# FROL256/ada-ray-tracer

Hardware: AMD Instinct MI355X
Metric: Mrays/s (higher is better)
Workload: dtype f32; 1 GPU; C4: synthetic 1000000 triangles + 3 sphere lights in the Cornell box, 1920x1080, PT_MIS depth 8, 2x2 AA, 256 spp per step; parallelism=pixel-tiles x1, bvh_width=4, bvh_nodes=383662, bvh_max_stack=36

## Files before the change

### ada-ray-tracer_amd/csrc/art_api.cpp

```cpp
#include <hip/hip_runtime.h>
#include <rccl/rccl.h>

#include <algorithm>
#include <chrono>
#include <cstdio>
#include <cstdlib>
#include <cstring>
#include <mutex>
#include <string>
#include <vector>

#include "art_api_internal.h"
#include "art_lbvh.h"

namespace art {

Ctx g_devs[kMaxDevices];
int g_ndev = 1;
Ctx* g_cur = &g_devs[0];
std::mutex g_mu;
static ncclComm_t g_comms[kMaxDevices];
static bool g_comms_ready = false;
static EventPairs g_reduce_pairs;
static double g_reduce_ms = 0.0; static int g_reduces = 0, g_reduce_path = 0;
// ... 530 lines not shown
        for (DevPaths& b : bank) { b.P = pn * sn; b.npix = pn; b.pixmap = (const uint32_t*)c.b_pixmap.p + px0; b.sample_base = (uint32_t)(c.spp + s0); }
        carve(bank, bank[0].P, p->max_depth, c.opt.trace_kernel == TRACE_COOP);
        int trial = 0, shade_per = c.opt.opt_shade_per ? c.opt.opt_shade_per : (c.auto_phase >= 4 ? c.auto_per : 4);
        if (c.opt.opt_shade_per == 0 && c.auto_phase < 3 && c.opt.trace_kernel == TRACE_COOP) {
          const int64_t Pb = (int64_t)pn * sn;
          if (c.auto_phase == 0) c.auto_phase = 1;
          else if (c.auto_phase == 1) { trial = 1; c.auto_ms[0] = 0.0; c.auto_P[0] = Pb; c.auto_phase = 2; }
          else if (Pb == c.auto_P[0]) { trial = 2; shade_per = 2; c.auto_ms[1] = 0.0; c.auto_P[1] = Pb; c.auto_phase = 3; }
          else if (++c.auto_redo > 3) { c.auto_per = 4; c.auto_phase = 4; }
          else { trial = 1; c.auto_gen += 1; c.auto_ms[0] = 0.0; c.auto_P[0] = Pb; }
        }
        const bool dedup = c.opt.camera_dedup && !c.opt.count_tests && c.opt.trace_kernel == TRACE_COOP;
        const int cam_u = p->aa_on ? 4 : 1;
        const int cam_n = dedup ? cam_u * pn : bank[0].P;
        c.camera_traced += (uint64_t)cam_n;
        if (c.opt.trace_kernel == TRACE_COOP) {
          if (!c.d_live) HIP_TRY(hipMalloc(&c.d_live, 32 * 18 * sizeof(int)));
          unsigned long long* const rays_b = c.opt.count_tests ? c.d_counters + CNT_TRACED : nullptr;
          bank[0].rec_mode = REC_EXT;
          DevPaths q = bank[0];
          q.slot_id = nullptr;
          q.cam_dedup = dedup ? cam_u : 0;
          DevPaths qgen = q; qgen.P = cam_n;
          if (!c.d_items) { HIP_TRY(hipMalloc(&c.d_items, 32 * sizeof(unsigned long long))); HIP_TRY(hipMemsetAsync(c.d_items, 0, 32 * sizeof(unsigned long long), c.stream)); }
          { EventPairs::Timer t; HIP_TRY(c.stage_pairs.begin(t, c.stream, ev_tag(2))); launch_raygen(c.stream, F, c.scene, qgen); }
          launch_bump(c.stream, c.d_counters + CNT_RAYS, rays_b, (unsigned long long)q.P);
          { const RecordQueue rq = {cam_n, nullptr, 1}; TraceLaunch t = launch; t.records = &rq; if (trace(q, cam_n, t)) return 1; }
          for (int b = 0; b < p->max_depth; ++b) {
            const int in = b & 1, out = in ^ 1;
            const DevPaths& qi = (b == 0) ? q : bank[in];
            const bool last = b + 1 >= p->max_depth;
            bank[out].rec_mode = (p->render_type == ART_PT_STUPID) ? REC_EXT : (last ? REC_SHADOW : REC_BOTH);
            int* const n_in = c.d_live + 32 * b; int* const n_out = c.d_live + 32 * (b + 1);
            HIP_TRY(hipMemsetAsync(n_out, 0, sizeof(int), c.stream));
            { EventPairs::Timer t; HIP_TRY(c.stage_pairs.begin(t, c.stream, ev_tag(1, trial)));
              launch_shade_compact(c.stream, F, c.scene, qi, bank[out], b, b == 0 ? nullptr : n_in, n_out,
                                   const_cast<uint32_t*>(bank[out].slot_id), c.d_counters + CNT_LOST, c.d_counters + CNT_RAYS, rays_b, shade_per); }
            if (b == 0 && c.inject_lost) { launch_bump(c.stream, c.d_counters + CNT_LOST, nullptr, 1ull); c.inject_lost = 0; }
            if (g_debug_live) {
              int n = -1; unsigned long long r0 = 0;
              (void)hipStreamSynchronize(c.stream); (void)hipMemcpy(&n, n_out, 4, hipMemcpyDeviceToHost); (void)hipMemcpy(&r0, c.d_counters + CNT_RAYS, 8, hipMemcpyDeviceToHost);
              std::fprintf(stderr, "stage %d: items out %d of %d, rays so far %llu\n", b, n, q.P, r0);
            }
            if (!last || p->render_type != ART_PT_STUPID) {
              const RecordQueue rq = {-1, n_out, bank[out].rec_mode == REC_BOTH ? 2 : 1};
              TraceLaunch t = launch; t.item_count = n_out; t.records = &rq;
              if (trace(bank[out], 2 * q.P, t)) return 1;
            }
          }
          const int last = p->max_depth & 1;
          EventPairs::Timer fold_timer;
          HIP_TRY(c.stage_pairs.begin(fold_timer, c.stream, ev_tag(3)));
          launch_resolve_last(c.stream, bank[last], c.d_live + 32 * p->max_depth, p->max_depth - 1);
          if (bank[last].fold_dense) launch_fold_levels(c.stream, F, bank[last], p->max_depth, c.d_live);
          else launch_fold(c.stream, F, bank[last]);
          launch_accumulate(c.stream, F, q, sn, accum_ptr());
          HIP_TRY(fold_timer.end());
          launch_acc_items(c.stream, c.d_live, p->max_depth, q.P, c.d_items);
          c.stage.batches += 1;
        } else {
          DevPaths q = bank[0];
          q.slot_id = nullptr;
          q.final_flags = q.flags;
          launch_raygen(c.stream, F, c.scene, q);
          for (int b = 0; b < p->max_depth; ++b) {
            if (trace(q, b == 0 ? q.P : 2 * q.P, launch)) return 1;
            launch_shade(c.stream, F, c.scene, q, b);
          }
          if (p->render_type != ART_PT_STUPID) { if (trace(q, 2 * q.P, launch)) return 1; }
          launch_finish(c.stream, F, q, p->max_depth - 1);
          launch_accumulate(c.stream, F, q, sn, accum_ptr());
        }
        HIP_TRY(hipGetLastError());
      }
    }
  }
  HIP_TRY(pass_timer.end());
  if (clock) HIP_TRY(hipLaunchHostFunc(c.stream, clock_cb, &clock->t1));
  c.spp += S;
  c.stats.samples += (uint64_t)npix * S;
  if (spp_inout) *spp_inout = c.spp;
  return 0;
}

static int synchronize_one();
int synchronize() {
  Dev0Guard guard;
  int rc = 0;
  for (int k = 0; k < g_ndev; ++k) { if (use_dev(k) || synchronize_one()) rc = 1; }
  if (g_devs[0].device_ready && !use_dev(0)) fold_reduce_events();
  return rc;
}
static int synchronize_one() {
  Ctx& c = g_ctx;
  if (!c.device_ready) return 0;
  HIP_TRY(hipStreamSynchronize(c.stream));
  HIP_TRY(c.pass_pairs.fold(true, [&c](float ms, uint8_t) { c.stats.pass_ms += ms; }));
  if (collect_timing()) return 1;
  if (sync_updates()) return 1;
  if (c.stats.lost_paths != c.lost_reported) {
    const uint64_t n = c.stats.lost_paths - c.lost_reported;
    c.lost_reported = c.stats.lost_paths;
    return fail("render self-check: " + std::to_string(n) + " path(s) lost by the wavefront stages (ArtStats::lost_paths); the image is not valid");
  }
  return 0;
}

// ... 475 lines not shown
int art_get_stage_stats(ArtStageStats* out) {
  std::lock_guard<std::mutex> lk(g_mu);
  if (!out) return fail("null ArtStageStats");
  if (synchronize()) return 1;
  *out = g_devs[0].stage;
  return 0;
}

int art_get_stats(ArtStats* out) {
  std::lock_guard<std::mutex> lk(g_mu);
  if (!out) return fail("null stats");
  if (synchronize()) return 1;
  *out = g_devs[0].stats;
  for (int k = 1; k < g_ndev; ++k) {
    const ArtStats& t = g_devs[k].stats;
    out->rays += t.rays; out->samples += t.samples; out->box_tests += t.box_tests; out->tri_tests += t.tri_tests;
    out->node_visits += t.node_visits; out->leaf_visits += t.leaf_visits; out->traced_rays += t.traced_rays;
    out->lost_paths += t.lost_paths;
    out->pass_ms = std::max(out->pass_ms, t.pass_ms);
  }
  return 0;
}

int art_get_camera_rays_traced(uint64_t* out) {
  std::lock_guard<std::mutex> lk(g_mu);
  if (!out) return fail("null camera ray count");
  *out = 0;
  for (int k = 0; k < g_ndev; ++k) *out += g_devs[k].camera_traced;
  return 0;
}

static int set_option_one(const std::string& n, int64_t value);
int art_set_option(const char* name, int64_t value) {
  std::lock_guard<std::mutex> lk(g_mu);
  if (!name) return fail("null option");
  const std::string n(name);
  Ctx* const saved = g_cur;
  int rc = 0;
  for (int k = 0; k < g_ndev && !rc; ++k) { g_cur = &g_devs[k]; rc = set_option_one(n, value); }
  g_cur = saved;
  return rc;
}
static int set_option_one(const std::string& n, int64_t value) {
  if (n == "trace_kernel") { if (value != TRACE_COOP && value != TRACE_SIMPLE) return fail("trace_kernel: 0 (cooperative) or 1 (simple)"); g_ctx.opt.trace_kernel = (int)value; }
  else if (n == "queue_segments") { if (value != 1 && value != 2 && value != 4 && value != 8) return fail("queue_segments: 1, 2, 4 or 8"); g_ctx.opt.queue_segments = (int)value; }
  else if (n == "batch_paths") { if (value < 1024 || value > (1ll << 27)) return fail("batch_paths: 1024..2^27 (2 rays per path slot; the trace kernel addresses a ray's 16-byte hit record by a 32-bit byte offset)"); g_ctx.opt.batch_paths = value; g_ctx.auto_phase = 0; g_ctx.auto_redo = 0; g_ctx.auto_gen += 1; }
  else if (n == "paths_spread") { if (value < -1 || value > 65536) return fail("paths_spread: chunk size in MB, 0 = off (plain hipMalloc), -1 = automatic"); g_ctx.opt.paths_spread_mb = (int)value; release_paths(g_ctx); }
  else if (n == "spread_fail_at") { g_ctx.spread_fail_at = (int)value; release_paths(g_ctx); }
  else if (n == "inject_lost") { g_ctx.inject_lost = value != 0; }
  else if (n == "blocks_per_cu") { g_ctx.opt.opt_blocks_per_cu = (int)value; g_ctx.blocks_per_cu = 0; }
  else if (n == "query_slice") { if (value < 1 || value > (1ll << 28)) return fail("query_slice: 1 .. 2^28 rays per slice of a device query"); g_ctx.opt.query_slice = value; }
  else if (n == "count_tests") { g_ctx.opt.count_tests = value != 0; }
  else if (n == "camera_dedup") { if (value != 0 && value != 1) return fail("camera_dedup: 0 (every sample's camera ray is traced) or 1 (each distinct camera ray once per batch)"); g_ctx.opt.camera_dedup = value != 0; }
  else if (n == "shadow_anyhit") { g_ctx.opt.shadow_anyhit = value != 0; }
  else if (n == "skip_null_shadow") { g_ctx.opt.skip_null_shadow = value != 0; }
  else if (n == "inst_coop") { g_ctx.opt.inst_coop = value != 0; }
  else if (n == "shade_per") { if (value != 0 && value != 2 && value != 4) return fail("shade_per: 0 (measured), 2 or 4"); g_ctx.opt.opt_shade_per = (int)value; }
  else if (n == "ray_chunk") { if (value < 16 || value > 4096 || (value & 15)) return fail("ray_chunk: a multiple of 16, 16..4096"); g_ctx.opt.ray_chunk = (int)value; }
  else if (n == "refill_min") { if (value < 1 || value > 8) return fail("refill_min: 1..8"); g_ctx.opt.refill_min = (int)value; }
  else if (n == "node_min") { if (value < 0 || value > 8) return fail("node_min: 1..8, 0 = automatic"); g_ctx.opt.node_min = (int)value; }
  else if (n == "bvh_width") { if (value != 4 && value != 8) return fail("bvh_width: 4 or 8"); g_ctx.opt.bvh_params.width = (int)value; }
  else if (n == "lds_stack_cap") { if (value < 0 || value > kStackEntries) return fail("lds_stack_cap: 0 (automatic) .. 160"); g_ctx.opt.lds_stack_cap = (int)value; }
  else if (n == "bvh_max_leaf") { if (value < 0 || value > kMaxLeafTris) return fail("bvh_max_leaf: 1..8, 0 = defaults"); g_ctx.opt.bvh_params.max_leaf = value ? (int)value : BvhBuildParams().max_leaf; g_ctx.opt.bvh_params.gpu_max_leaf = (int)value; }
  else if (n == "inst_open") { if (value < 0 || value > 4096) return fail("inst_open: 1 .. 4096 entry points per instance, 0 = chosen from the instances' overlap"); g_ctx.opt.bvh_params.inst_open = (int)value; }
  else if (n == "bvh_spatial_splits") { g_ctx.opt.bvh_params.spatial_alpha = value ? 1.0e-5f : -1.0f; }
  else if (n == "bvh_builder") { if (value < 0 || value > 3) return fail("bvh_builder: 0 host SAH, 1 GPU LBVH, 2 GPU PLOC, 3 GPU SAH"); g_ctx.opt.bvh_params.builder = (int)value; }
  else if (n == "bvh_ploc_radius") { if (value < 1 || value > 64) return fail("bvh_ploc_radius: 1..64"); g_ctx.opt.bvh_params.ploc_radius = (int)value; }
  else if (n == "bvh_leaf_base_milli") { g_ctx.opt.bvh_params.leaf_base = (float)value / 1000.0f; }
  else if (n == "bvh_tri_cost_milli") { g_ctx.opt.bvh_params.tri_cost = (float)value / 1000.0f; }
  else if (n == "bvh_node_cost_milli") { g_ctx.opt.bvh_params.node_cost = (float)value / 1000.0f; }
  else return fail("unknown option " + n);
  return 0;
}

const char* art_last_error(void) { t_err = g_err; return t_err.c_str(); }

void art_shutdown(void) { std::lock_guard<std::mutex> lk(g_mu); shutdown(); }

}
```

### ada-ray-tracer_amd/csrc/art_api_internal.h

```cpp
#pragma once
#include <hip/hip_runtime.h>
#include <mutex>
#include <string>
#include <vector>
#include "../../include/art_hip.h"
#include "art_event_pairs.h"
#include "art_host_scene.h"
#include "art_kernels.h"

namespace art {

constexpr int kMaxDevices = 16;
constexpr int kCursorInts = 32 * 9;

struct DevBuf {
  void* p = nullptr; size_t bytes = 0;
  std::vector<hipMemGenericAllocationHandle_t> chunks; size_t chunk_bytes = 0, reserved = 0;
  void release();
};

struct UpdateLane {
  EventPairs pairs;
  hipEvent_t ready_ev = nullptr, done_ev = nullptr;
  DevBuf b_stage;
  bool unread = false;
  uint64_t bad_last = 0; bool bad_reported = true;
};

struct Options {
  int trace_kernel = TRACE_COOP;
  int64_t batch_paths = 128ll << 20;
  int opt_blocks_per_cu = 0;
  bool count_tests = false;
  bool camera_dedup = true;
  int node_min = 0;
  int refill_min = 2;
  int queue_segments = 8;
  int ray_chunk = 48;
  bool shadow_anyhit = true;
  bool skip_null_shadow = false;
  bool inst_coop = true;
  int opt_shade_per = 0;
  int lds_stack_cap = 0;
  int paths_spread_mb = -1;
  int64_t query_slice = 1ll << 24;
  BvhBuildParams bvh_params;
};

enum Counter {
  CNT_RAYS = 0,
  CNT_STATS = 3, CNT_TRACED = 7,
  CNT_NODE_ITERS = 8, CNT_LEAF_ITERS = 9, CNT_WAVE_ITERS = 10, CNT_LOST = 15, kCounters = 16
};

struct Ctx {
  int device = -1; bool device_ready = false; int num_cus = 0; int lds_per_cu = 160 * 1024; std::string arch;
  hipStream_t stream = nullptr;
  hipStream_t own_stream = nullptr;
  bool scene_ready = false;
  HostScene host_scene;
  DevScene scene;
  DevScene* d_scene = nullptr;
  DevBuf b_spheres, b_sphere_mat, b_lights, b_materials, b_bf_pos, b_bf_nrm, b_bf_uv, b_bf_idx, b_nodes, b_qnodes, b_tris, b_qtris, b_m_shade;
  int bvh_stack_bound = 8;
  int width = 0, height = 0, spp = 0;
  int rank = 0, nranks = 1, tile = 32, npix_local = 0;
  DevBuf b_inst, b_tlas_nodes, b_tlas_tris, b_blas_nodes, b_blas_tris;
  DevBuf b_accum, b_screen, b_stage, b_pixmap, b_paths, b_rays, b_ids, b_queue, b_ovf;
  DevBuf b_query;
  hipEvent_t q_ev[2] = {nullptr, nullptr};
  struct RefitPlan {
    bool ready = false;
    DevBuf b_idx, b_levels, b_tight, b_bad;
    std::vector<int> level_off;
    uint64_t bad_total = 0;
    UpdateLane lane;
  } refit;
  struct MovePlan {
    bool ready = false;
    DevBuf b_plan, b_work;
    MoveArgs args = MoveArgs();
    std::vector<int> level_off; const int32_t* levels = nullptr;
    bool small_entries = false;
    UpdateLane lane;
    struct Mesh { int32_t tri_base = -1, n_recs = 0, shade_base = 0, n_prims = 0; int64_t nverts = 0; const int32_t* idx = nullptr; int level_first = 0, level_end = 0; };
    std::vector<Mesh> meshes;
    std::vector<int> blas_level_off; const int32_t* blas_levels = nullptr;
    UpdateLane refit_lane;
  } move;
  int* d_live = nullptr;
  DevBuf b_reduced;
// ... 82 lines not shown
```

### ada-ray-tracer_amd/csrc/art_kernels.h

```cpp
#pragma once
#include <hip/hip_runtime.h>
#include "art_shade.h"
#include "art_qnode.h"
#include "art_instanced.h"

namespace art {

enum { TRACE_COOP = 0, TRACE_SIMPLE = 1 };

struct TraceArgs {
  int32_t n_rays;
  int32_t stack_entries;
  int32_t width;
  int32_t instanced;
  int32_t stack_overflow;
  int32_t segments;
  int32_t node_min;
  int32_t refill_min;
  const float* ray_ox; const float* ray_oy; const float* ray_oz;
  const float* ray_dx; const float* ray_dy; const float* ray_dz;
  const float* ray_tfar;
  float4* rec;
  const float* sh_min; int32_t shadow_begin;
  DevHit* hit;
  const DevInstance* inst; int32_t inst_shift;
  float* sh_t;
  const float* nodes; const uint32_t* qnodes; const float* tris; const float* qtris; int32_t n_tris;
  int32_t chunk;
  int* cursor;
  int* queue; int* queue_count;
  int32_t queue_fixed; const int* queue_items; int32_t queue_mul;
  int* ovf_queue; int* ovf_count;
  unsigned long long* stats;
  unsigned long long* live_rays;
  const int* item_count;
};

constexpr int kTraceRecBytes = 64;

void launch_raygen(hipStream_t st, const DevFrame& F, const DevScene& S, const DevPaths& Q);
void launch_bump(hipStream_t st, unsigned long long* a, unsigned long long* b, unsigned long long n);
void launch_acc_items(hipStream_t st, const int* live, int depth, int P, unsigned long long* items);
void launch_shade(hipStream_t st, const DevFrame& F, const DevScene& S, const DevPaths& Q, int bounce);
void launch_finish(hipStream_t st, const DevFrame& F, const DevPaths& Q, int last_level);
void launch_shade_compact(hipStream_t st, const DevFrame& F, const DevScene& S, const DevPaths& Qi, const DevPaths& Qo, int bounce,
                          const int* n_in, int* n_out, uint32_t* slot_out, unsigned long long* lost, unsigned long long* rays_a, unsigned long long* rays_b,
                          int per = 0);
void launch_resolve_last(hipStream_t st, const DevPaths& Q, const int* n, int last_level);
void launch_fold(hipStream_t st, const DevFrame& F, const DevPaths& Q);
void launch_fold_levels(hipStream_t st, const DevFrame& F, const DevPaths& Q, int max_depth, const int* counts);
void launch_accumulate(hipStream_t st, const DevFrame& F, const DevPaths& Q, int samples_in_batch, float* accum);
void launch_resolve(hipStream_t st, const float* accum, int n_pixels, float norm_c, uint32_t* screen);
void launch_debug(hipStream_t st, const DevFrame& F, const DevScene& S, const DevPaths& Q, float* accum, int32_t* prim_index, int32_t* mat_id, int32_t* prim_type);
void launch_to_xmajor_f3(hipStream_t st, const float* src, float* dst, int w, int h);
void launch_to_xmajor_u32(hipStream_t st, const uint32_t* src, uint32_t* dst, int w, int h);
void launch_from_xmajor_f3(hipStream_t st, const float* src, float* dst, int w, int h);
void launch_trace_instanced(hipStream_t st, const InstScene& T, const float* o, const float* d, const float* tfar, int n, InstHit* out);
void launch_pad_tris(hipStream_t st, const float* src12, float* dst16, int n);
void launch_add_f32(hipStream_t st, const float* src, float* dst, size_t n);
size_t trace_coop_lds_bytes(int stack_entries, int width);
void launch_trace(hipStream_t st, const DevScene* d_scene, const TraceArgs& A, int kernel, bool stats, int grid_blocks);
void launch_analytic(hipStream_t st, const DevScene& scene, const TraceArgs& A, bool stats);
int  trace_coop_blocks_per_cu(int stack_entries, int width);

constexpr int kArtHitWords = 11;
struct QueryArgs {
  int32_t n;
  const float* o3; const float* d3;
  const float* tnear; const float* tfar;
  float *ox, *oy, *oz, *dx, *dy, *dz, *tf;
  float* shm;
  DevHit* hit;
  uint32_t* out;
  uint8_t* occluded;
};
void launch_query_pack(hipStream_t st, const QueryArgs& Q);
void launch_query_finalize(hipStream_t st, const DevScene& S, const QueryArgs& Q);
void launch_query_occluded(hipStream_t st, const QueryArgs& Q);

constexpr float kRefitMaxCoord = 1.0e18f;
struct RefitArgs {
  const float* pos3f; const float* nrm3f;
  const int32_t* idx;
  int64_t nverts; int32_t n_prims, n_recs;
  float* tris; float* qtris; float* m_shade;
  unsigned long long* bad;
  float* nodes; QNode* qnodes;
  float* tight;
  int32_t width; float inflate_rel, inflate_abs;
};
void launch_refit_tris(hipStream_t st, const RefitArgs& R);
void launch_refit_level(hipStream_t st, const RefitArgs& R, const int32_t* level_nodes, int n);

struct GatherArgs {
  const float* pos3f; const int32_t* idx;
  int64_t nverts; int32_t n_prims;
  float* tri9;
  unsigned long long* bad;
};
void launch_gather_tri9(hipStream_t st, const GatherArgs& G);
void launch_tree_cost(hipStream_t st, const float* nodes, int n_nodes, int width, double* sums4);

struct MoveArgs {
// ... 36 lines not shown
```

### ada-ray-tracer_amd/csrc/art_kernels.hip

```cpp
#include <hip/hip_runtime.h>
#include <algorithm>
#include <type_traits>
#include "art_kernels.h"

namespace art {

template <int CTRL>
__device__ __forceinline__ int dpp_i(int v) { return __builtin_amdgcn_update_dpp(0, v, CTRL, 0xf, 0xf, true); }

constexpr int DPP_XOR1 = 0xB1;
constexpr int DPP_XOR2 = 0x4E;
constexpr int DPP_XOR3 = 0x1B;
constexpr int DPP_HALF_MIRROR = 0x141;

__device__ __forceinline__ int xor4_i(int v) { return dpp_i<DPP_XOR3>(dpp_i<DPP_HALF_MIRROR>(v)); }

template <int G> __device__ __forceinline__ int group_rank_g(int key);
template <> __device__ __forceinline__ int group_rank_g<4>(int key) {
  int r = 0;
  r += (dpp_i<DPP_XOR1>(key) < key);
  r += (dpp_i<DPP_XOR2>(key) < key);
  r += (dpp_i<DPP_XOR3>(key) < key);
  return r;
}
// ... 735 lines not shown
    const int r = wave * 64 + lane;
    const int n_all_k = s_nall[k], n_keep_k = s_nkeep[k], out0_k = s_out0[k];
    const int wo = r < n_keep_k ? base + out0_k + r : -1;
    if (r < n_all_k) {
      const uint2 hk = s_hint[k * 256 + r];
      const int w = c0 + k * 256 + (int)(hk.y & 255u);
      ItemHint ih; ih.key = hk.x; ih.mat = (hk.y & 256u) ? (int32_t)(hk.y >> 9) : -1;
      StageCtx cy = tables;
      if (staged) {
        const int nk = min(64, max(0, n_keep_k - wave * 64)), per = (Qo.rec_mode == REC_BOTH) ? 2 : 1;
        const size_t first = (size_t)per * (size_t)(base + out0_k + wave * 64);
        cy.stage = s_stage[wave]; cy.stage_pitch = kStagePitch; cy.stage_item = lane; cy.stage_count = nk; cy.lost = lost;
        cy.rec_base[0] = first; cy.rec_base[1] = (per == 2) ? first + (size_t)nk : first;
      }
      n_rays += shade_item(F, S, Qi, Qo, w, wo, bounce, lost, cy, &ih, CAMERA ? 1 : 0, 1);
    }
  }
  ART_TPROBE(tables.tprobe, 68);
#if defined(ART_TIME_PROBE)
  __syncthreads();
  if (threadIdx.x < 64 && s_tacc[threadIdx.x] != 0) atomicAdd(&g_lane_probe[2 * 64 + threadIdx.x], s_tacc[threadIdx.x]);
#endif
  if (Qo.rec != nullptr && rays_a != nullptr) {
    for (int off = 32; off > 0; off >>= 1) n_rays += __shfl_xor(n_rays, off);
    if (lane == 0 && n_rays) atomicAdd(&s_rays, n_rays);
    __syncthreads();
    if (threadIdx.x == 0 && s_rays) { atomicAdd(rays_a, (unsigned long long)s_rays); if (rays_b) atomicAdd(rays_b, (unsigned long long)s_rays); }
  }
}

__global__ void k_bump(unsigned long long* a, unsigned long long* b, unsigned long long n) { *a += n; if (b) *b += n; }
__global__ void k_acc_items(const int* live, int depth, int P, unsigned long long* items) {
  unsigned long long in = (unsigned long long)P;
  for (int b = 0; b < depth && b < 16; ++b) { const unsigned long long out = (unsigned long long)live[32 * (b + 1)]; items[b] += in; items[16 + b] += out; in = out; }
}

__global__ __launch_bounds__(256) void k_resolve_last(const DevPaths Q, const int* __restrict__ n_ptr, int last_level) {
  const int w = blockIdx.x * blockDim.x + threadIdx.x;
  if (w < *n_ptr) resolve_last_shadow(Q, w, last_level);
}
__global__ __launch_bounds__(256) void k_fold(const DevFrame F, const DevPaths Q) {
  const int slot = blockIdx.x * blockDim.x + threadIdx.x;
  if (slot < Q.P) fold_slot(F, Q, slot);
}

__global__ __launch_bounds__(256) void k_fold_level(const DevFrame F, const DevPaths Q, int level, int deepest, const int* __restrict__ n_ptr,
                                                    const float* __restrict__ nxt_r, const float* __restrict__ nxt_g, const float* __restrict__ nxt_b,
                                                    float* __restrict__ cur_r, float* __restrict__ cur_g, float* __restrict__ cur_b) {
  const int w = blockIdx.x * blockDim.x + threadIdx.x;
  const int n = n_ptr ? *n_ptr : Q.P;
  if (w < n) fold_level_item(F, Q, level, w, deepest != 0, nxt_r, nxt_g, nxt_b, cur_r, cur_g, cur_b);
}

__global__ __launch_bounds__(256) void k_finish(const DevFrame F, const DevPaths Q, int last_level) {
  const int slot = blockIdx.x * blockDim.x + threadIdx.x;
  if (slot < Q.P) finish_slot(F, Q, slot, last_level);
}

__global__ __launch_bounds__(256) void k_accumulate(const DevFrame F, const DevPaths Q, int samples_in_batch, float* accum) {
  const int pl = blockIdx.x * blockDim.x + threadIdx.x;
  if (pl < Q.npix) accumulate_pixel(F, Q, pl, samples_in_batch, accum);
}

__global__ __launch_bounds__(256) void k_resolve(const float* accum, int n_pixels, float norm_c, uint32_t* screen) {
  const int i = blockIdx.x * blockDim.x + threadIdx.x;
  if (i < n_pixels) screen[i] = resolve_pixel(mk3(accum[3 * (size_t)i], accum[3 * (size_t)i + 1], accum[3 * (size_t)i + 2]), norm_c);
}

__global__ __launch_bounds__(256) void k_debug(const DevFrame F, const DevScene S, const DevPaths Q, float* accum,
                                               int32_t* prim_index, int32_t* mat_id, int32_t* prim_type) {
  const int slot = blockIdx.x * blockDim.x + threadIdx.x;
  if (slot >= Q.P) return;
  uint32_t pixel, sample;
  slot_to_sample(Q, slot, pixel, sample);
  const DevHit hq = Q.hit[slot];
  const uint32_t key = hq.key;
  f3 col = mk3(0.0f, 0.0f, 0.0f);
  int32_t pi = -1, mi = -1, pt = -1;
  if (key != KEY_MISS) {
    const f3 o = mk3(Q.ray_ox[slot], Q.ray_oy[slot], Q.ray_oz[slot]), d = mk3(Q.ray_dx[slot], Q.ray_dy[slot], Q.ray_dz[slot]);
    const Surface sf = surface_at(S, o, d, hq.t, key, hq.u, hq.v);
    col = debug_palette(sf.mat_id);
    mi = sf.mat_id; pi = (int32_t)(key & KEY_INDEX_MASK);
    const uint32_t cls = key & ~KEY_INDEX_MASK;
    pt = (cls == KEY_CORNELL) ? 0 : (cls == KEY_SPHERE) ? 1 : (cls == KEY_QUAD) ? 3 : 2;
  }
  accum[3 * (size_t)pixel] = col.x; accum[3 * (size_t)pixel + 1] = col.y; accum[3 * (size_t)pixel + 2] = col.z;
  if (prim_index) prim_index[pixel] = pi;
  if (mat_id) mat_id[pixel] = mi;
  if (prim_type) prim_type[pixel] = pt;
}

__global__ __launch_bounds__(256) void k_to_xmajor_f3(const float* src_rowmajor, float* dst_xmajor, int w, int h) {
  const int i = blockIdx.x * blockDim.x + threadIdx.x;
  if (i >= w * h) return;
  const int x = i / h, y = i - x * h;
  const size_t s = (size_t)y * w + x;
  dst_xmajor[3 * (size_t)i] = src_rowmajor[3 * s]; dst_xmajor[3 * (size_t)i + 1] = src_rowmajor[3 * s + 1]; dst_xmajor[3 * (size_t)i + 2] = src_rowmajor[3 * s + 2];
}
__global__ __launch_bounds__(256) void k_to_xmajor_u32(const uint32_t* src_rowmajor, uint32_t* dst_xmajor, int w, int h) {
  const int i = blockIdx.x * blockDim.x + threadIdx.x;
  if (i >= w * h) return;
  const int x = i / h, y = i - x * h;
  dst_xmajor[i] = src_rowmajor[(size_t)y * w + x];
}
__global__ __launch_bounds__(256) void k_from_xmajor_f3(const float* src_xmajor, float* dst_rowmajor, int w, int h) {
// ... 14 lines not shown
__global__ __launch_bounds__(256) void k_add_f32(const float* __restrict__ src, float* __restrict__ dst, size_t n) {
  const size_t i = (size_t)blockIdx.x * blockDim.x + threadIdx.x;
  if (i < n) dst[i] = src[i] + dst[i];
}

static inline int blocks_for(int n) { return (n + 255) / 256; }

void launch_raygen(hipStream_t st, const DevFrame& F, const DevScene& S, const DevPaths& Q) {
  hipLaunchKernelGGL(k_raygen, dim3(blocks_for(Q.P)), dim3(256), 0, st, F, S, Q);
}
void launch_shade(hipStream_t st, const DevFrame& F, const DevScene& S, const DevPaths& Q, int bounce) {
  hipLaunchKernelGGL(k_shade, dim3(blocks_for(Q.P)), dim3(256), 0, st, F, S, Q, bounce);
}
#if defined(ART_LANE_PROBE)
__global__ void k_probe_on(int v) { g_lane_probe_on = v; }
#endif
void launch_shade_compact(hipStream_t st, const DevFrame& F, const DevScene& S, const DevPaths& Qi, const DevPaths& Qo, int bounce,
                          const int* n_in, int* n_out, uint32_t* slot_out, unsigned long long* lost, unsigned long long* rays_a, unsigned long long* rays_b,
                          int per) {
  const bool camera = Qi.synth0 && Qi.slot_id == nullptr;
  const int per_now = (per == 2) ? 2 : kShadePerThread;
  const dim3 grid((Qi.P + 256 * per_now - 1) / (256 * per_now));
#if defined(ART_LANE_PROBE)
  hipLaunchKernelGGL(k_probe_on, dim3(1), dim3(1), 0, st, 1);
#endif
  ShadeKernArgs A; A.F = F; A.S = S; A.Qi = Qi; A.Qo = Qo; A.bounce = bounce; A.n_in_ptr = n_in; A.n_out_ptr = n_out; A.slot_out = slot_out; A.lost = lost; A.rays_a = rays_a; A.rays_b = rays_b;
  if (per_now == 2) {
    if (camera) hipLaunchKernelGGL((k_shade_compact<2, true>), grid, dim3(256), 0, st, A);
    else hipLaunchKernelGGL((k_shade_compact<2, false>), grid, dim3(256), 0, st, A);
  } else {
    if (camera) hipLaunchKernelGGL((k_shade_compact<kShadePerThread, true>), grid, dim3(256), 0, st, A);
    else hipLaunchKernelGGL((k_shade_compact<kShadePerThread, false>), grid, dim3(256), 0, st, A);
  }
#if defined(ART_LANE_PROBE)
  hipLaunchKernelGGL(k_probe_on, dim3(1), dim3(1), 0, st, 0);
#endif
}
void launch_acc_items(hipStream_t st, const int* live, int depth, int P, unsigned long long* items) { hipLaunchKernelGGL(k_acc_items, dim3(1), dim3(1), 0, st, live, depth, P, items); }
void launch_bump(hipStream_t st, unsigned long long* a, unsigned long long* b, unsigned long long n) { hipLaunchKernelGGL(k_bump, dim3(1), dim3(1), 0, st, a, b, n); }
void launch_resolve_last(hipStream_t st, const DevPaths& Q, const int* n, int last_level) {
  hipLaunchKernelGGL(k_resolve_last, dim3(blocks_for(Q.P)), dim3(256), 0, st, Q, n, last_level);
}
void launch_fold(hipStream_t st, const DevFrame& F, const DevPaths& Q) {
  hipLaunchKernelGGL(k_fold, dim3(blocks_for(Q.P)), dim3(256), 0, st, F, Q);
}
void launch_fold_levels(hipStream_t st, const DevFrame& F, const DevPaths& Q, int max_depth, const int* counts) {
  for (int k = max_depth - 1; k >= 0; --k) {
    float* cur[3] = {(k & 1) ? Q.term_r : Q.rad_r, (k & 1) ? Q.term_g : Q.rad_g, (k & 1) ? Q.term_b : Q.rad_b};
    const float* nxt[3] = {(k & 1) ? Q.rad_r : Q.term_r, (k & 1) ? Q.rad_g : Q.term_g, (k & 1) ? Q.rad_b : Q.term_b};
    hipLaunchKernelGGL(k_fold_level, dim3(blocks_for(Q.P)), dim3(256), 0, st, F, Q, k, k == max_depth - 1 ? 1 : 0, k == 0 ? nullptr : counts + 32 * k,
                       nxt[0], nxt[1], nxt[2], cur[0], cur[1], cur[2]);
  }
}
void launch_finish(hipStream_t st, const DevFrame& F, const DevPaths& Q, int last_level) {
  hipLaunchKernelGGL(k_finish, dim3(blocks_for(Q.P)), dim3(256), 0, st, F, Q, last_level);
}
void launch_accumulate(hipStream_t st, const DevFrame& F, const DevPaths& Q, int samples_in_batch, float* accum) {
  hipLaunchKernelGGL(k_accumulate, dim3(blocks_for(Q.npix)), dim3(256), 0, st, F, Q, samples_in_batch, accum);
}
void launch_resolve(hipStream_t st, const float* accum, int n_pixels, float norm_c, uint32_t* screen) {
  hipLaunchKernelGGL(k_resolve, dim3(blocks_for(n_pixels)), dim3(256), 0, st, accum, n_pixels, norm_c, screen);
}
void launch_debug(hipStream_t st, const DevFrame& F, const DevScene& S, const DevPaths& Q, float* accum, int32_t* prim_index, int32_t* mat_id, int32_t* prim_type) {
  hipLaunchKernelGGL(k_debug, dim3(blocks_for(Q.P)), dim3(256), 0, st, F, S, Q, accum, prim_index, mat_id, prim_type);
}
void launch_to_xmajor_f3(hipStream_t st, const float* src, float* dst, int w, int h) {
  hipLaunchKernelGGL(k_to_xmajor_f3, dim3(blocks_for(w * h)), dim3(256), 0, st, src, dst, w, h);
}
void launch_to_xmajor_u32(hipStream_t st, const uint32_t* src, uint32_t* dst, int w, int h) {
  hipLaunchKernelGGL(k_to_xmajor_u32, dim3(blocks_for(w * h)), dim3(256), 0, st, src, dst, w, h);
}
void launch_from_xmajor_f3(hipStream_t st, const float* src, float* dst, int w, int h) {
  hipLaunchKernelGGL(k_from_xmajor_f3, dim3(blocks_for(w * h)), dim3(256), 0, st, src, dst, w, h);
}

void launch_trace_instanced(hipStream_t st, const InstScene& T, const float* o, const float* d, const float* tfar, int n, InstHit* out) {
  hipLaunchKernelGGL(k_trace_instanced, dim3((n + 63) / 64), dim3(64), 0, st, T, o, d, tfar, n, out);
}

void launch_pad_tris(hipStream_t st, const float* src, float* dst, int n) {
  hipLaunchKernelGGL(k_pad_tris, dim3((unsigned)(((size_t)n * 16 + 255) / 256)), dim3(256), 0, st, src, dst, n);
}

void launch_add_f32(hipStream_t st, const float* src, float* dst, size_t n) {
  hipLaunchKernelGGL(k_add_f32, dim3((unsigned)((n + 255) / 256)), dim3(256), 0, st, src, dst, n);
}

size_t trace_coop_lds_bytes(int stack_entries, int width) { return (size_t)4 * (64 / width) * (stack_entries + 3) * sizeof(uint2); }

void launch_analytic(hipStream_t st, const DevScene& S, const TraceArgs& A, bool stats) {
  TraceArgs B = A;
  if (!stats) B.stats = nullptr;
  hipLaunchKernelGGL(k_analytic, dim3((A.n_rays + kAnalyticChunk - 1) / kAnalyticChunk), dim3(256), 0, st, S, B);
}

void launch_trace(hipStream_t st, const DevScene* S, const TraceArgs& A, int kernel, bool stats, int grid_blocks) {
  if (kernel == TRACE_SIMPLE) {
    hipLaunchKernelGGL(k_count_live, dim3((A.n_rays + kAnalyticChunk - 1) / kAnalyticChunk), dim3(256), 0, st, A);
    if (stats) hipLaunchKernelGGL(k_trace_simple<true>, dim3(blocks_for(A.n_rays)), dim3(256), 0, st, S, A);
    else hipLaunchKernelGGL(k_trace_simple<false>, dim3(blocks_for(A.n_rays)), dim3(256), 0, st, S, A);
    return;
  }
  if (A.n_tris <= 0) return;
  if (A.instanced == 2) {
    const int blocks = std::max(1, std::min(grid_blocks * 4, 65535));
    if (stats) hipLaunchKernelGGL(k_trace_inst<true>, dim3(blocks), dim3(256), 0, st, S, A);
// ... 53 lines not shown
```

### ada-ray-tracer_amd/csrc/art_shade.h

```cpp
#pragma once
#include "art_isect.h"

namespace art {

constexpr float kGEpsilon = 1.0e-5f;
constexpr float kGEpsilonDiv = 1.0e-20f;
constexpr float kEpsDiv = 1.0e-20f;
constexpr float kEpsCos = 1.0e-6f;
constexpr float kPhongClamp = 0x1.921eaep+0f;

struct StageCtx {
  const DevSphere* spheres = nullptr; const DevLight* lights = nullptr; const DevMaterial* materials = nullptr;
  const ART_LDS DevSphere* lds_spheres = nullptr; const ART_LDS DevLight* lds_lights = nullptr;
  Rec4* stage = nullptr; int stage_pitch = 0; int stage_item = 0;
  int stage_count = 0; size_t rec_base[2] = {0, 0};
  bool hot_layout = false;
  unsigned long long* tprobe = nullptr;
  unsigned long long* lost = nullptr;
};

template <class T = float> ART_HD T* hotf(const DevPaths& q, int field) { return reinterpret_cast<T*>(q.hot + (size_t)field * (size_t)q.stride); }
ART_HD float* cold_e(const DevPaths& q, int c, int level) { return q.cold + ((size_t)c * (size_t)(q.depth + 1) + (size_t)level) * (size_t)q.P; }
ART_HD float* cold_w(const DevPaths& q, int c, int level) { return q.cold + ((size_t)3 * (size_t)(q.depth + 1) + (size_t)c * (size_t)q.depth + (size_t)level) * (size_t)q.P; }
ART_HD int32_t* cold_child(const DevPaths& q, int level) { return reinterpret_cast<int32_t*>(q.cold + ((size_t)3 * (size_t)(q.depth + 1) + (size_t)3 * (size_t)q.depth + (size_t)level) * (size_t)q.P); }
// ... 775 lines not shown
    if (mode != REC_SHADOW) emit_ray(s, qo, (size_t)wo, rec_slot(mode, wo, false), alive, no, nd, kInfinity, -1.0f, cx, blocks ? cx.stage_item : per * cx.stage_item, 0);
    ART_TPROBE(cx.tprobe, 76);
    if (mode != REC_EXT) emit_ray(s, qo, (batch || qo.sh_t) ? (size_t)(kShadowWord | (uint32_t)wo) : so_i, rec_slot(mode, wo, true), shadow, so, sd, s_tfar, qo.shadow_rule ? sh_min : -1.0f, cx, blocks ? cx.stage_item : per * cx.stage_item + (per - 1), 1);
    ART_TPROBE(cx.tprobe, 77);
    if (lost != nullptr && ((mode == REC_SHADOW && alive) || (mode == REC_EXT && shadow))) {
#if defined(__HIP_DEVICE_COMPILE__)
      atomicAdd(lost, 1ull);
#endif
    }
    return (alive ? 1 : 0) + (shadow ? 1 : 0);
  }
  qo.ray_tfar[wo] = alive ? kInfinity : -1.0f;
  qo.ray_tfar[so_i] = shadow ? s_tfar : -1.0f;
  if (shadow) {
    qo.ray_ox[so_i] = so.x; qo.ray_oy[so_i] = so.y; qo.ray_oz[so_i] = so.z;
    qo.ray_dx[so_i] = sd.x; qo.ray_dy[so_i] = sd.y; qo.ray_dz[so_i] = sd.z;
  }
  return (alive ? 1 : 0) + (shadow ? 1 : 0);
}

ART_HD void shade_slot(const DevFrame& f, const DevScene& s, const DevPaths& q, int slot, int bounce) { (void)shade_item(f, s, q, q, slot, slot, bounce); }

ART_HD void resolve_last_shadow(const DevPaths& q, int w, int last_level) {
  const uint32_t fl = q.flags[w];
  if (!(fl & FLAG_SHADOW_PENDING)) return;
  const int slot = item_slot(q, w);
  float hs_t;
  if (q.sh_t) hs_t = q.sh_t[w];
  else { const DevHit hs = q.hit[(size_t)q.P + (size_t)w]; hs_t = (hs.key != KEY_MISS) ? hs.t : -1.0f; }
  const bool in_shadow = (hs_t >= 0.0f) && (hs_t > q.sh_min_t[w]);
  if (q.fold_dense) {
    if (in_shadow) { const size_t li = (size_t)(last_level + 1) * (size_t)q.P + (size_t)w; q.e_r[li] = 0.0f; q.e_g[li] = 0.0f; q.e_b[li] = 0.0f; }
  } else {
    const size_t li = (size_t)last_level * (size_t)q.P + (size_t)slot;
    q.e_r[li] = in_shadow ? 0.0f : q.cand_r[w];
    q.e_g[li] = in_shadow ? 0.0f : q.cand_g[w];
    q.e_b[li] = in_shadow ? 0.0f : q.cand_b[w];
  }
  q.flags[w] = fl & ~FLAG_SHADOW_PENDING;
}

ART_HD void fold_slot(const DevFrame& f, const DevPaths& q, int slot) {
  const int levels = (int)(q.final_flags[slot] >> 8);
  f3 L = mk3(q.term_r[slot], q.term_g[slot], q.term_b[slot]);
  for (int k = levels - 1; k >= 0; --k) {
    const size_t li = (size_t)k * q.P + slot;
    const f3 w = mk3(q.w_r[li], q.w_g[li], q.w_b[li]);
    if (f.render_type == PT_STUPID) L = w * L;
    else L = mk3(q.e_r[li], q.e_g[li], q.e_b[li]) + w * L;
  }
  q.rad_r[slot] = L.x; q.rad_g[slot] = L.y; q.rad_b[slot] = L.z;
}

ART_HD void fold_level_item(const DevFrame& f, const DevPaths& q, int level, int w, bool deepest,
                            const float* nxt_r, const float* nxt_g, const float* nxt_b, float* cur_r, float* cur_g, float* cur_b) {
  const size_t lw = (size_t)level * (size_t)q.P + (size_t)w;
  const int32_t cw = q.child[lw];
  const int32_t kind = (cw >> 28) & 3, c = cw & kFoldIndexMask;
  f3 L = mk3(q.w_r[lw], q.w_g[lw], q.w_b[lw]);
  if (kind != 1) {
    const f3 wv = L;
    const bool has = (kind == 0);
    const f3 Ln = (has && !deepest) ? mk3(nxt_r[c], nxt_g[c], nxt_b[c]) : mk3(0.0f, 0.0f, 0.0f);
    if (f.render_type == PT_STUPID) L = wv * Ln;
    else {
      const size_t le = (size_t)(level + 1) * (size_t)q.P + (size_t)c;
      const bool counts = has && (deepest || ((q.child[le] >> 30) & 1) == 0);
      const f3 ev = counts ? mk3(q.e_r[le], q.e_g[le], q.e_b[le]) : mk3(0.0f, 0.0f, 0.0f);
      L = ev + wv * Ln;
    }
  }
  cur_r[w] = L.x; cur_g[w] = L.y; cur_b[w] = L.z;
}

ART_HD void finish_slot(const DevFrame& f, const DevPaths& q, int slot, int last_level) {
  resolve_last_shadow(q, slot, last_level);
  fold_slot(f, q, slot);
}

ART_HD void accumulate_pixel(const DevFrame& f, const DevPaths& q, int pl, int samples_in_batch, float* accum ) {
  const uint32_t pixel = q.pixmap ? q.pixmap[pl] : (uint32_t)pl;
  float* a = accum + 3 * (size_t)pixel;
  f3 acc = mk3(a[0], a[1], a[2]);
  if (f.aa_on) {
    for (int t = 0; t + 3 < samples_in_batch; t += 4) {
      f3 color = ld3(f.background);
      for (int i = 0; i < 4; ++i) {
        const size_t si = (size_t)(t + i) * q.npix + pl;
        color = color + mk3(q.rad_r[si], q.rad_g[si], q.rad_b[si]);
      }
      acc = color + acc;
    }
  } else {
    for (int t = 0; t < samples_in_batch; ++t) {
      const size_t si = (size_t)t * q.npix + pl;
      acc = mk3(q.rad_r[si], q.rad_g[si], q.rad_b[si]) + acc;
    }
  }
  a[0] = acc.x; a[1] = acc.y; a[2] = acc.z;
}

ART_HD uint32_t ada_round_u32(float v) {
  if (!(v > 0.0f)) return 0u;
  uint32_t u = (uint32_t)v;
  if (v - (float)u >= 0.5f) u += 1u;
  return u;
}

ART_HD uint32_t resolve_pixel(f3 acc, float norm_c) {
  f3 rgb = acc * norm_c;
  rgb.x = apow(rgb.x, 1.0f / 2.0f); rgb.y = apow(rgb.y, 1.0f / 2.0f); rgb.z = apow(rgb.z, 1.0f / 2.0f);
  const uint32_t r = ada_round_u32(amin(rgb.x, 1.0f) * 255.0f);
  const uint32_t g = ada_round_u32(amin(rgb.y, 1.0f) * 255.0f);
  const uint32_t b = ada_round_u32(amin(rgb.z, 1.0f) * 255.0f);
  return r | (g << 8) | (b << 16);
}

ART_HD f3 debug_palette(int32_t mat_id) {
  switch (mat_id % 8) {
    case 0: return mk3(0.5f, 0.0f, 0.0f);   case 1: return mk3(0.0f, 0.5f, 0.0f);
    case 2: return mk3(0.0f, 0.0f, 0.5f);   case 3: return mk3(0.5f, 0.5f, 0.5f);
    case 4: return mk3(0.5f, 0.5f, 0.0f);   case 5: return mk3(0.5f, 0.0f, 0.5f);
    case 6: return mk3(0.0f, 0.5f, 0.5f);   default: return mk3(0.75f, 0.75f, 0.75f);
  }
// ... 4 lines not shown
```

Measured before the change: 1893 Mrays/s.

## Fold all path levels in one kernel by chasing child links per slot

```diff
diff --git a/ada-ray-tracer_amd/csrc/art_api.cpp b/ada-ray-tracer_amd/csrc/art_api.cpp
--- a/ada-ray-tracer_amd/csrc/art_api.cpp
+++ b/ada-ray-tracer_amd/csrc/art_api.cpp
@@ -606,7 +606,8 @@
           EventPairs::Timer fold_timer;
           HIP_TRY(c.stage_pairs.begin(fold_timer, c.stream, ev_tag(3)));
           launch_resolve_last(c.stream, bank[last], c.d_live + 32 * p->max_depth, p->max_depth - 1);
-          if (bank[last].fold_dense) launch_fold_levels(c.stream, F, bank[last], p->max_depth, c.d_live);
+          if (bank[last].fold_dense && c.opt.fold_chain) launch_fold_chain(c.stream, F, bank[last], p->max_depth);
+          else if (bank[last].fold_dense) launch_fold_levels(c.stream, F, bank[last], p->max_depth, c.d_live);
           else launch_fold(c.stream, F, bank[last]);
           launch_accumulate(c.stream, F, q, sn, accum_ptr());
           HIP_TRY(fold_timer.end());
@@ -1188,6 +1189,7 @@
   else if (n == "query_slice") { if (value < 1 || value > (1ll << 28)) return fail("query_slice: 1 .. 2^28 rays per slice of a device query"); g_ctx.opt.query_slice = value; }
   else if (n == "count_tests") { g_ctx.opt.count_tests = value != 0; }
   else if (n == "camera_dedup") { if (value != 0 && value != 1) return fail("camera_dedup: 0 (every sample's camera ray is traced) or 1 (each distinct camera ray once per batch)"); g_ctx.opt.camera_dedup = value != 0; }
+  else if (n == "fold_chain") { if (value != 0 && value != 1) return fail("fold_chain: 0 (one fold launch per level) or 1 (every level in one pass)"); g_ctx.opt.fold_chain = value != 0; }
   else if (n == "shadow_anyhit") { g_ctx.opt.shadow_anyhit = value != 0; }
   else if (n == "skip_null_shadow") { g_ctx.opt.skip_null_shadow = value != 0; }
   else if (n == "inst_coop") { g_ctx.opt.inst_coop = value != 0; }
diff --git a/ada-ray-tracer_amd/csrc/art_api_internal.h b/ada-ray-tracer_amd/csrc/art_api_internal.h
--- a/ada-ray-tracer_amd/csrc/art_api_internal.h
+++ b/ada-ray-tracer_amd/csrc/art_api_internal.h
@@ -37,6 +37,7 @@
   int refill_min = 2;
   int queue_segments = 8;
   int ray_chunk = 48;
+  bool fold_chain = true;
   bool shadow_anyhit = true;
   bool skip_null_shadow = false;
   bool inst_coop = true;
diff --git a/ada-ray-tracer_amd/csrc/art_kernels.h b/ada-ray-tracer_amd/csrc/art_kernels.h
--- a/ada-ray-tracer_amd/csrc/art_kernels.h
+++ b/ada-ray-tracer_amd/csrc/art_kernels.h
@@ -49,6 +49,7 @@
 void launch_resolve_last(hipStream_t st, const DevPaths& Q, const int* n, int last_level);
 void launch_fold(hipStream_t st, const DevFrame& F, const DevPaths& Q);
 void launch_fold_levels(hipStream_t st, const DevFrame& F, const DevPaths& Q, int max_depth, const int* counts);
+void launch_fold_chain(hipStream_t st, const DevFrame& F, const DevPaths& Q, int max_depth);
 void launch_accumulate(hipStream_t st, const DevFrame& F, const DevPaths& Q, int samples_in_batch, float* accum);
 void launch_resolve(hipStream_t st, const float* accum, int n_pixels, float norm_c, uint32_t* screen);
 void launch_debug(hipStream_t st, const DevFrame& F, const DevScene& S, const DevPaths& Q, float* accum, int32_t* prim_index, int32_t* mat_id, int32_t* prim_type);
diff --git a/ada-ray-tracer_amd/csrc/art_kernels.hip b/ada-ray-tracer_amd/csrc/art_kernels.hip
--- a/ada-ray-tracer_amd/csrc/art_kernels.hip
+++ b/ada-ray-tracer_amd/csrc/art_kernels.hip
@@ -811,6 +811,34 @@
   if (w < n) fold_level_item(F, Q, level, w, deepest != 0, nxt_r, nxt_g, nxt_b, cur_r, cur_g, cur_b);
 }
 
+template <int MAXD>
+__global__ __launch_bounds__(256) void k_fold_chain(const DevFrame F, const DevPaths Q, int depth) {
+  const int s = blockIdx.x * blockDim.x + threadIdx.x;
+  if (s >= Q.P) return;
+  const size_t P = (size_t)Q.P;
+  FoldRec rec[MAXD];
+  int n = 0, w = s;
+  bool go = true;
+  int32_t cw = Q.child[s];
+#pragma unroll
+  for (int k = 0; k < MAXD; ++k) {
+    if (go && k < depth) {
+      const bool deepest = (k + 1 == depth);
+      const int32_t c = cw & kFoldIndexMask;
+      const bool down = ((cw >> 28) & 3) == 0 && !deepest;
+      const int32_t cn = down ? Q.child[(size_t)(k + 1) * P + (size_t)c] : 0;
+      rec[k] = fold_level_load(F, Q, k, w, cw, fold_asks_successor(F, cw, deepest) && ((cn >> 30) & 1) != 0);
+      n = k + 1; go = down; w = c; cw = cn;
+    }
+  }
+  f3 L = mk3(0.0f, 0.0f, 0.0f);
+#pragma unroll
+  for (int k = MAXD - 1; k >= 0; --k) {
+    if (k < n) L = fold_level_step(F, rec[k], L);
+  }
+  Q.rad_r[s] = L.x; Q.rad_g[s] = L.y; Q.rad_b[s] = L.z;
+}
+
 __global__ __launch_bounds__(256) void k_finish(const DevFrame F, const DevPaths Q, int last_level) {
   const int slot = blockIdx.x * blockDim.x + threadIdx.x;
   if (slot < Q.P) finish_slot(F, Q, slot, last_level);
@@ -931,6 +959,10 @@
                        nxt[0], nxt[1], nxt[2], cur[0], cur[1], cur[2]);
   }
 }
+void launch_fold_chain(hipStream_t st, const DevFrame& F, const DevPaths& Q, int max_depth) {
+  if (max_depth <= 8) hipLaunchKernelGGL(k_fold_chain<8>, dim3(blocks_for(Q.P)), dim3(256), 0, st, F, Q, max_depth);
+  else hipLaunchKernelGGL(k_fold_chain<16>, dim3(blocks_for(Q.P)), dim3(256), 0, st, F, Q, max_depth);
+}
 void launch_finish(hipStream_t st, const DevFrame& F, const DevPaths& Q, int last_level) {
   hipLaunchKernelGGL(k_finish, dim3(blocks_for(Q.P)), dim3(256), 0, st, F, Q, last_level);
 }
diff --git a/ada-ray-tracer_amd/csrc/art_shade.h b/ada-ray-tracer_amd/csrc/art_shade.h
--- a/ada-ray-tracer_amd/csrc/art_shade.h
+++ b/ada-ray-tracer_amd/csrc/art_shade.h
@@ -851,24 +851,34 @@
   q.rad_r[slot] = L.x; q.rad_g[slot] = L.y; q.rad_b[slot] = L.z;
 }
 
+struct FoldRec { f3 w, e; int32_t kind; };
+ART_HD FoldRec fold_level_load(const DevFrame& f, const DevPaths& q, int level, int w, int32_t cw, bool succ_shadowed) {
+  const size_t lw = (size_t)level * (size_t)q.P + (size_t)w;
+  const int32_t kind = (cw >> 28) & 3, c = cw & kFoldIndexMask;
+  FoldRec r; r.kind = kind; r.w = mk3(q.w_r[lw], q.w_g[lw], q.w_b[lw]); r.e = mk3(0.0f, 0.0f, 0.0f);
+  if (kind != 1 && f.render_type != PT_STUPID) {
+    const size_t le = (size_t)(level + 1) * (size_t)q.P + (size_t)c;
+    const bool counts = (kind == 0) && !succ_shadowed;
+    if (counts) r.e = mk3(q.e_r[le], q.e_g[le], q.e_b[le]);
+  }
+  return r;
+}
+ART_HD f3 fold_level_step(const DevFrame& f, const FoldRec& r, f3 Ln) {
+  if (r.kind == 1) return r.w;
+  if (f.render_type == PT_STUPID) return r.w * Ln;
+  return r.e + r.w * Ln;
+}
+ART_HD bool fold_asks_successor(const DevFrame& f, int32_t cw, bool deepest) {
+  return ((cw >> 28) & 3) == 0 && !deepest && f.render_type != PT_STUPID;
+}
 ART_HD void fold_level_item(const DevFrame& f, const DevPaths& q, int level, int w, bool deepest,
                             const float* nxt_r, const float* nxt_g, const float* nxt_b, float* cur_r, float* cur_g, float* cur_b) {
-  const size_t lw = (size_t)level * (size_t)q.P + (size_t)w;
-  const int32_t cw = q.child[lw];
+  const int32_t cw = q.child[(size_t)level * (size_t)q.P + (size_t)w];
   const int32_t kind = (cw >> 28) & 3, c = cw & kFoldIndexMask;
-  f3 L = mk3(q.w_r[lw], q.w_g[lw], q.w_b[lw]);
-  if (kind != 1) {
-    const f3 wv = L;
-    const bool has = (kind == 0);
-    const f3 Ln = (has && !deepest) ? mk3(nxt_r[c], nxt_g[c], nxt_b[c]) : mk3(0.0f, 0.0f, 0.0f);
-    if (f.render_type == PT_STUPID) L = wv * Ln;
-    else {
-      const size_t le = (size_t)(level + 1) * (size_t)q.P + (size_t)c;
-      const bool counts = has && (deepest || ((q.child[le] >> 30) & 1) == 0);
-      const f3 ev = counts ? mk3(q.e_r[le], q.e_g[le], q.e_b[le]) : mk3(0.0f, 0.0f, 0.0f);
-      L = ev + wv * Ln;
-    }
-  }
+  const bool succ_shadowed = fold_asks_successor(f, cw, deepest) && ((q.child[(size_t)(level + 1) * (size_t)q.P + (size_t)c] >> 30) & 1) != 0;
+  const FoldRec r = fold_level_load(f, q, level, w, cw, succ_shadowed);
+  const f3 Ln = (kind == 0 && !deepest) ? mk3(nxt_r[c], nxt_g[c], nxt_b[c]) : mk3(0.0f, 0.0f, 0.0f);
+  const f3 L = fold_level_step(f, r, Ln);
   cur_r[w] = L.x; cur_g[w] = L.y; cur_b[w] = L.z;
 }
 
diff --git a/profiles/fold_chain/ab.py b/profiles/fold_chain/ab.py
--- /dev/null
+++ b/profiles/fold_chain/ab.py
@@ -0,0 +1,60 @@
+import argparse
+import json
+import os
+import statistics
+import sys
+import time
+
+ROOT = os.path.dirname(os.path.dirname(os.path.dirname(os.path.abspath(__file__))))
+sys.path.insert(0, ROOT)
+import __graft_entry__ as ge
+
+
+def main():
+    ap = argparse.ArgumentParser()
+    ap.add_argument("--rounds", type=int, default=3)
+    ap.add_argument("--steps", type=int, default=2)
+    ap.add_argument("--warmup", type=int, default=2)
+    ap.add_argument("--tris", type=int, default=1000000)
+    ap.add_argument("--width", type=int, default=1920)
+    ap.add_argument("--height", type=int, default=1080)
+    ap.add_argument("--vthreads", type=int, default=64)
+    args = ap.parse_args()
+    art = ge.load_package()
+    from ada_ray_tracer_amd import scenes
+    be = art.Backend(0)
+    be.upload_scene(scenes.synthetic_scene(args.tris, 4))
+    be.resize(args.width, args.height)
+    prm = art.Backend.pass_params(art.PT_MIS, True, 8, args.vthreads, seed=1)
+    spp = 0
+    for _ in range(args.warmup):
+        spp = be.render_pass_device(prm, spp)
+    be.synchronize()
+    res = {0: [], 1: []}
+    for rnd in range(args.rounds):
+        for chain in (0, 1):
+            be.set_option("fold_chain", chain)
+            s0, g0 = be.stats(), be.stage_stats()
+            t0 = time.perf_counter()
+            for _ in range(args.steps):
+                spp = be.render_pass_device(prm, spp)
+            be.synchronize()
+            ms = (time.perf_counter() - t0) * 1e3 / args.steps
+            s1, g1 = be.stats(), be.stage_stats()
+            batches = g1.batches - g0.batches
+            row = {"round": rnd, "fold_chain": chain, "ms_per_step": round(ms, 2), "trace_ms_per_step": round((s1.trace_ms - s0.trace_ms) / args.steps, 2),
+                   "fold_ms_per_batch": round((g1.fold_ms - g0.fold_ms) / batches, 4), "shade_ms_per_step": round((g1.shade_ms - g0.shade_ms) / args.steps, 2),
+                   "batches_per_step": batches // args.steps, "rays_per_step": (s1.rays - s0.rays) // args.steps}
+            res[chain].append(row)
+            print(json.dumps(row), flush=True)
+    be.set_option("fold_chain", 1)
+    fields = ("ms_per_step", "trace_ms_per_step", "fold_ms_per_batch", "shade_ms_per_step")
+    med = {k: {f: statistics.median(r[f] for r in rows) for f in fields} for k, rows in res.items()}
+    spread = {k: {f: round(max(r[f] for r in rows) - min(r[f] for r in rows), 4) for f in fields} for k, rows in res.items()}
+    print(json.dumps({"median": {"fold_chain=1": med[1], "fold_chain=0": med[0]}, "spread": {"fold_chain=1": spread[1], "fold_chain=0": spread[0]},
+                      "fold_ms_per_batch_delta": round(med[1]["fold_ms_per_batch"] - med[0]["fold_ms_per_batch"], 4)}))
+    be.shutdown()
+
+
+if __name__ == "__main__":
+    main()
```

Result: no change. 1897 Mrays/s, median of 6 (+0.2%).
